# oxfordcontrol/COSMO.jl

Measured on AMD Instinct MI355X. Metric: ADMM iterations/sec (fp64) at fixed (n,m,nnz,cone), higher is better.
Workload: dtype f64

## Files before the change

cosmo.jl_amd/csrc/psd_polar.hip:

```cpp
#include "psd_internal.h"
#include <math.h>
#include <stdlib.h>
#include <string.h>
#include <algorithm>
#include <mutex>

#define PK 16
#ifndef POLAR_PREFETCH_DEPTH
#define POLAR_PREFETCH_DEPTH 2
#endif
#define PLD 80

struct PolarCone {
  int idx;
  int off, d, kind;
  int ts;
  int sk;
  int skg, skc;
  int ld;
  long long woff;
};

struct BatchCone { long long woff; int off, d, kind, ld, idx, ts; };

// ... 25 lines not shown
  real* W = nullptr;
  real* parts = nullptr;
  real* nrm = nullptr;
  int k_lift = REAL_IS_FLOAT ? 5 : 9;
  int max_rounds = 2;
  int rescale = 1;
  int batch_occ = 3;
  real tol_factor = 8.0;
  PolarDev* dev = nullptr;
  PolarDev seen;
  long long launches[4] = {0, 0, 0, 0};
  int streamk = 0;
  real* sk_scratch = nullptr;
  SkSync* sk_sync = nullptr;
  int sk_gmax = 0;
  unsigned sk_base = 0, sk_epoch = 0;
  int products_last_large = 0, products_last_batch = 0;
  std::vector<BatchCone> bcones;
  BatchCone* d_bcones = nullptr;
  int4* d_btiles = nullptr;
  int nbtiles = 0, nbtiles96 = 0;
  int speculate = 0;
  int* gate_host = nullptr;
  int batch_wave = 0;
  int batch_ragged = 1;
  void* d_rtiles = nullptr;
  int nrtiles = 0;
  int dataflow = 0;
  void* d_df_tiles = nullptr;
  int* d_df_cone_nt = nullptr;
  unsigned* d_df_sync = nullptr;
  int df_xoff[9] = {0, 0, 0, 0, 0, 0, 0, 0, 0};
  int df_grid = 0;
  long long df_launches = 0, df_timed = 0;
  int df_nprod = 0;
  double df_seconds = 0.0;
  hipEvent_t df_ev[2] = {nullptr, nullptr};
  int df_ev_pending = 0;
  void* h_rtiles = nullptr;
  void* rep_host = nullptr;
  void* d_rtiles_rep = nullptr;
  int nrep = 0;
  long long repair_launch_tiles = 0, repair_trains = 0;
  double batch_flops_performed = 0.0, batch_flops_useful = 0.0;
  int batch_ts96 = 0;
  real* BW = nullptr;
  real* bparts = nullptr;
  real* bnrm = nullptr;
  int* bgate = nullptr;
  int adapt = 0;
  int compact_repair = 1;
  std::vector<int> bk, bstreak, bm;
  int* d_lgate = nullptr;
  int* d_ubuf = nullptr;
  int* bgate_host = nullptr;
  int lgate_kmax = -1;
  long long depth_fail = 0, depth_down = 0, depth_proj = 0;
  int seen_proj_batch = 0;
  std::vector<int> lk, lstreak, lm;
  int seen_proj_large = 0;
  double wprod_last = 0.0;
};
#define POLAR_LIFT_CAP 18

extern "C" int32_t cosmo_hip_polar_schedule(int32_t k_lift, double* abc, int32_t* nsteps) {
  if (k_lift < 0 || k_lift > 64 || !nsteps) return COSMO_HIP_ERR_INVALID;
// ... 513 lines not shown
  t_first = RT_NOW();
#endif
  if (DEPTH == 1) {
    for (int kb = 0; kb + 1 < nk; kb += 2) {
      R_LOAD(r[0], kb + 1)
      R_COMPUTE(0)
      R_STORE(r[0], 1)
      __syncthreads();
      if (kb + 2 >= nk) break;
      R_LOAD(r[0], kb + 2)
      R_COMPUTE(1)
      R_STORE(r[0], 0)
      __syncthreads();
    }
  } else
  for (int kb = 0; kb + 1 < nk; kb += 2) {
    if (kb + 2 < nk) R_LOAD(r[0], kb + 2)
    R_COMPUTE(0)
    R_STORE(r[DEPTH - 1], 1)
    __syncthreads();
    if (kb + 2 >= nk) break;
    if (kb + 3 < nk) R_LOAD(r[DEPTH - 1], kb + 3)
    R_COMPUTE(1)
    R_STORE(r[0], 0)
    __syncthreads();
  }
  pre_last();
  if ((nk - 1) & 1) R_COMPUTE(1) else R_COMPUTE(0)
#undef R_LOAD
#undef R_STORE
#undef R_COMPUTE
}

template <int EPI, int OCC, bool SC1 = false, class Hook>
__device__ __forceinline__ void ragged_tile(const RTile& td, real* __restrict__ W, int ia, int ib, int icin, int ic, real alpha, real beta, real* smem, Hook pre_last) {
  const unsigned long long t_start = RT_NOW();
  unsigned long long t_first = t_start;
  (void)t_first;
#ifdef POLAR_LAB_TIMING
  const unsigned long long w_start = (threadIdx.x == 0) ? wall_clock64() : 0ull;
#endif
  const int ld = td.ld;
  const long long n2 = (long long)ld * ld;
  real* base = W + td.woff;
  const real* A = base + ia * n2;
  const real* B = base + ib * n2;
  const real* Cin = base + icin * n2;
  real* C = base + ic * n2;
  const int ei = td.ext & 255, ej = (td.ext >> 8) & 255, diag = (td.ext >> 16) & 1;
  const int nblk = diag ? ei * (ei + 1) / 2 : ei * ej;
  const int wv = __builtin_amdgcn_readfirstlane(threadIdx.x >> 6), lane = threadIdx.x & 63;
  int oa[4], ob[4];
  int nsl = 0;
#pragma unroll
  for (int sl = 0; sl < 4; ++sl) {
    const int q = wv + 4 * sl;
    int bi = 0, bj = 0;
    if (q < nblk) {
      nsl = sl + 1;
      if (diag) { bj = (q >= 6) ? 3 : (q >= 3) ? 2 : (q >= 1) ? 1 : 0; bi = q - bj * (bj + 1) / 2; }
      else { bj = q / ei; bi = q - bj * ei; }
    }
    oa[sl] = 16 * bi; ob[sl] = 16 * bj;
  }
  v4d acc[4];
#pragma unroll
// ... 3 lines not shown
  const int i0 = td.i0, j0 = td.j0;
  __amdgpu_buffer_rsrc_t rs = __builtin_amdgcn_make_buffer_rsrc((void*)base, 0, SC1 ? (int)(4 * n2 * (long long)sizeof(real)) : 0, 0x00020000);
  const int offA = (int)(ia * n2) + td.i0, offB = (int)(ib * n2) + td.j0;
#ifndef POLAR_LAB_NO_MAINLOOP
#define R_MAINLOOP(NSL_, SAME_) symm_mainloop_r<NSL_, (OCC >= 4 ? 1 : 2), SC1, SAME_>(A, B, ld, i0, j0, nk, smem, acc, oa, ob, pre_last, rs, offA, offB RT_ARG)
#ifndef POLAR_LAB_TWO_PANELS
  if (diag && offA == offB) {
    switch (nsl) {
      case 3: R_MAINLOOP(3, true); break;
      case 2: R_MAINLOOP(2, true); break;
      case 1: R_MAINLOOP(1, true); break;
      default: R_MAINLOOP(0, true); break;
    }
  } else
#endif
  switch (nsl) {
    case 4: R_MAINLOOP(4, false); break;
    case 3: R_MAINLOOP(3, false); break;
    case 2: R_MAINLOOP(2, false); break;
    case 1: R_MAINLOOP(1, false); break;
    default: R_MAINLOOP(0, false); break;
  }
#undef R_MAINLOOP
#else
  (void)A; (void)B; (void)nk; (void)pre_last;
#endif
#ifdef POLAR_LAB_NO_EPILOGUE
  if (lane == 0) C[(long long)j0 * ld + i0 + wv] = acc[0][0] + acc[1][0] + acc[2][0] + acc[3][0];
  return;
#endif
  const unsigned long long t_main = RT_NOW();
  (void)t_main; (void)t_start;
  (void)xi; (void)xj;
  {
    const int lj = lane & 15;
#pragma unroll
    for (int sl = 0; sl < 4; ++sl) {
      if (sl < nsl) {
        const int j = ob[sl] + lj;
        const bool dblk = diag && (oa[sl] == ob[sl]);
        real v[4];
        if (EPI == 1) {
          real c[4];
#pragma unroll
          for (int q = 0; q < 4; ++q) {
            const int i = oa[sl] + ACC_ROW(lane, q);
            const bool ok = !(dblk && i > j);
            const real* cp = Cin + (ok ? (long long)(i0 + i) * ld + j0 + j : 0);
            c[q] = SC1 ? __hip_atomic_load(cp, __ATOMIC_RELAXED, __HIP_MEMORY_SCOPE_AGENT) : *cp;
            if (!ok) c[q] = R(0.0);
          }
#pragma unroll
          for (int q = 0; q < 4; ++q) v[q] = alpha * acc[sl][q] + beta * c[q];
        } else {
#pragma unroll
          for (int q = 0; q < 4; ++q) v[q] = acc[sl][q];
        }
#pragma unroll
        for (int q = 0; q < 4; ++q) {
          const int i = oa[sl] + ACC_ROW(lane, q);
          if (!(dblk && i > j)) C[(long long)(j0 + j) * ld + i0 + i] = v[q];
        }
#pragma unroll
        for (int q = 0; q < 4; ++q) {
          const int i = oa[sl] + ACC_ROW(lane, q);
          if (!(dblk && i >= j)) C[(long long)(i0 + i) * ld + j0 + j] = v[q];
        }
      }
    }
  }
#ifdef POLAR_LAB_TIMING
  { const unsigned long long t_end = RT_NOW();
    RT_ADD(0, t_start); RT_ADD(1, t_first); RT_ADD(2, t_main); RT_ADD(3, t_end); RT_ADD(4, nk);
    if (threadIdx.x == 0 && blockIdx.x < RT_MAXT) g_rtw[blockIdx.x] = wall_clock64() - w_start; }
#endif
}

template <int EPI, int OCC>
__global__ __launch_bounds__(256) __attribute__((amdgpu_waves_per_eu(OCC, OCC))) void k_symm_gemm_batch_r(const Ctl* __restrict__ ctl, int guard, const int* __restrict__ gate,
                                                         const RTile* __restrict__ tiles, const BatchCone* __restrict__ cones, real* __restrict__ W,
                                                         int ia, int ib, int icin, int ic, real alpha, real beta) {
  extern __shared__ real smem[];
  const RTile td = tiles[blockIdx.x];
  const int halted = guard ? ctl->halt : 0;
  if (halted) return;
  if (td.cone < 0) return;
  if (gate && !gate[td.cone]) return;
  (void)cones;
  ragged_tile<EPI, OCC>(td, W, ia, ib, icin, ic, alpha, beta, smem, []() {});
}

struct DfProd { int ia, ib, icin, ic, epi, pad; real alpha, beta; };
#define DF_MAX_PROD 64
struct DfArgs { DfProd prod[DF_MAX_PROD]; int nprod; int xoff[9]; };
#define DF_SYNC_DONE 144
__device__ __forceinline__ unsigned df_xcc_id() { unsigned x; asm volatile("s_getreg_b32 %0, hwreg(HW_REG_XCC_ID)" : "=s"(x)); return x & 7u; }
__device__ __forceinline__ unsigned df_ld(const unsigned* p) { return __hip_atomic_load(p, __ATOMIC_RELAXED, __HIP_MEMORY_SCOPE_AGENT); }
#define DF_RMW(ptr) __hip_atomic_fetch_add((ptr), 1u, __ATOMIC_RELAXED, __HIP_MEMORY_SCOPE_AGENT)
template <int OCC>
__global__ __launch_bounds__(256) __attribute__((amdgpu_waves_per_eu(OCC, OCC))) void k_polar_dataflow(Ctl* __restrict__ ctl, int guard, const RTile* __restrict__ tiles,
                                                         const int* __restrict__ cone_nt, unsigned* __restrict__ sync, real* __restrict__ W, const DfArgs a) {
  extern __shared__ real smem[];
  __shared__ unsigned s_item;
  __shared__ int s_fail;
  if (guard && ctl->halt) return;
  const int x = (int)df_xcc_id();
  const int x0 = a.xoff[x];
  const unsigned n_x = (unsigned)(a.xoff[x + 1] - x0);
  const unsigned total = n_x * (unsigned)a.nprod;
  const bool wave0 = __builtin_amdgcn_readfirstlane(threadIdx.x >> 6) == 0;
  if (wave0) { if (threadIdx.x == 0) { s_fail = 0; s_item = (n_x > 0) ? DF_RMW(sync + 16 * x) : 0u; } }
  int prev_cone = -1;
  unsigned nxt = 0;
  bool first = true;
  for (;;) {
    if (wave0) {
      if (threadIdx.x == 0) {
        if (prev_cone >= 0) (void)DF_RMW(sync + DF_SYNC_DONE + prev_cone);
        if (!first) s_item = nxt;
      }
    }
    first = false;
    __syncthreads();
    const unsigned item = __builtin_amdgcn_readfirstlane(s_item);
    if (item >= total) break;
    const unsigned p = item / n_x, t = item - p * n_x;
    const RTile td = tiles[x0 + t];
    if (p > 0) {
      if (wave0) {
        if (threadIdx.x == 0) {
          const unsigned target = p * (unsigned)cone_nt[td.cone];
          const unsigned* cnt = sync + DF_SYNC_DONE + td.cone;
          long sp = 0;
          while (df_ld(cnt) < target) {
            __builtin_amdgcn_s_sleep(1);
            ++sp;
            if ((sp & 255) == 0 && df_ld(sync + 128)) { s_fail = 1; break; }
            if (sp > (1L << 20)) { s_fail = 1; __hip_atomic_store(sync + 128, 1u, __ATOMIC_RELAXED, __HIP_MEMORY_SCOPE_AGENT); ctl->error = COSMO_HIP_ERR_HIP; break; }
          }
        }
      }
      __syncthreads();
      if (__builtin_amdgcn_readfirstlane(s_fail)) break;
    }
    const DfProd pr = a.prod[p];
    auto hook = [&]() { if (wave0) { if (threadIdx.x == 0) nxt = DF_RMW(sync + 16 * x); } };
    if (pr.epi) ragged_tile<1, OCC, true>(td, W, pr.ia, pr.ib, pr.icin, pr.ic, pr.alpha, pr.beta, smem, hook);
    else ragged_tile<0, OCC, true>(td, W, pr.ia, pr.ib, pr.icin, pr.ic, pr.alpha, pr.beta, smem, hook);
    asm volatile("s_waitcnt vmcnt(0)" ::: "memory");
    __syncthreads();
    prev_cone = td.cone;
  }
}
#ifdef POLAR_LAB_TIMING
}
extern "C" void cosmo_dbg_ragged_timing(unsigned long long* out ) {
  (void)hipDeviceSynchronize();
  (void)hipMemcpyFromSymbol(out, HIP_SYMBOL(g_rt), sizeof(unsigned long long) * RT_MAXT * 5);
}
extern "C" void cosmo_dbg_ragged_wall(unsigned long long* out ) {
  (void)hipDeviceSynchronize();
  (void)hipMemcpyFromSymbol(out, HIP_SYMBOL(g_rtw), sizeof(unsigned long long) * RT_MAXT);
}
namespace {
#endif

#define WT_DEPTH 4
#define WT_SPITCH 66
template <int EPI>
__global__ __launch_bounds__(64) __attribute__((amdgpu_waves_per_eu(2, 2))) void k_symm_gemm_batch_w(const Ctl* __restrict__ ctl, int guard, const int* __restrict__ gate,
                                                         const int4* __restrict__ tiles, const BatchCone* __restrict__ cones, real* __restrict__ W,
                                                         int ia, int ib, int icin, int ic, real alpha, real beta) {
  if (guard && ctl->halt) return;
  const int4 td = tiles[blockIdx.x];
  if (td.x < 0) return;
  if (gate && !gate[td.x]) return;
  __shared__ real strip[16 * WT_SPITCH];
  const BatchCone bc = cones[td.x];
  const int ld = bc.ld;
  const long long n2 = (long long)ld * ld;
  real* base = W + bc.woff;
  const real* __restrict__ A = base + ia * n2;
  const real* __restrict__ B = base + ib * n2;
  const real* __restrict__ Cin = base + icin * n2;
  real* __restrict__ C = base + ic * n2;
// ... 423 lines not shown
      std::vector<int4> tl;
      if (getenv("COSMO_HIP_POLAR_BATCH_FLAT")) {
        for (int ci : order) {
          if (q->bcones[ci].ts != ts) continue;
          const int nt = q->bcones[ci].ld / ts;
          for (int tj = 0; tj < nt; ++tj) for (int ti = 0; ti <= tj; ++ti) tl.push_back(int4{ci, ti, tj, 0});
        }
      } else {
        std::vector<std::vector<int4>> xl(8);
        long long load[8] = {0, 0, 0, 0, 0, 0, 0, 0};
        for (int ci : order) {
          if (q->bcones[ci].ts != ts) continue;
          const int nt = q->bcones[ci].ld / ts;
          int x = 0;
          for (int t = 1; t < 8; ++t) if (load[t] < load[x]) x = t;
          for (int tj = 0; tj < nt; ++tj) for (int ti = 0; ti <= tj; ++ti) xl[x].push_back(int4{ci, ti, tj, 0});
          load[x] += (long long)nt * (nt + 1) / 2 * q->bcones[ci].ld;
        }
        size_t maxlen = 0;
        for (int x = 0; x < 8; ++x) maxlen = std::max(maxlen, xl[x].size());
        tl.assign(8 * maxlen, int4{-1, 0, 0, 0});
        for (int x = 0; x < 8; ++x) for (size_t sl = 0; sl < xl[x].size(); ++sl) tl[8 * sl + x] = xl[x][sl];
      }
      count[cls] = (int)tl.size();
      tiles.insert(tiles.end(), tl.begin(), tl.end());
    }
    q->nbtiles = count[0]; q->nbtiles96 = count[1];
    if (const char* e = getenv("COSMO_HIP_POLAR_BATCH_RAGGED")) q->batch_ragged = atoi(e) ? 1 : 0;
    if (q->batch_ts96 || q->batch_wave) q->batch_ragged = 0;
    q->batch_flops_performed = q->batch_flops_useful = 0.0;
    for (const BatchCone& bc : q->bcones) q->batch_flops_useful += (double)bc.d * bc.d * (bc.d + 1.0);
    if (q->batch_ragged) {
      std::vector<std::vector<RTile>> xl(8);
      long long load[8] = {0, 0, 0, 0, 0, 0, 0, 0};
      for (int ci : order) {
        const BatchCone& bc = q->bcones[ci];
        const int nb16 = (bc.d + 15) / 16, nt = (nb16 + 3) / 4;
        std::vector<int> start(nt + 1, 0);
        for (int t = 0; t < nt; ++t) start[t + 1] = start[t] + nb16 / nt + (t < nb16 % nt ? 1 : 0);
        int x = 0;
        for (int t = 1; t < 8; ++t) if (load[t] < load[x]) x = t;
        for (int tj = 0; tj < nt; ++tj)
          for (int ti = 0; ti <= tj; ++ti) {
            const int ei = start[ti + 1] - start[ti], ej = start[tj + 1] - start[tj], dg = (ti == tj) ? 1 : 0;
            RTile rt; rt.cone = ci; rt.i0 = 16 * start[ti]; rt.j0 = 16 * start[tj]; rt.ext = ei | (ej << 8) | (dg << 16);
            rt.ld = bc.ld; rt.d = bc.d; rt.woff = bc.woff;
            if (rt.i0 + 64 > bc.ld || rt.j0 + 64 > bc.ld) return cosmo_fail(h, COSMO_HIP_ERR_INVALID, "ragged tile exceeds the leading dimension");
            xl[x].push_back(rt);
            const int nblk = dg ? ei * (ei + 1) / 2 : ei * ej, slots = (nblk + 3) / 4;
            load[x] += (long long)slots * nb16;
            q->batch_flops_performed += 2.0 * 256.0 * nblk * 16.0 * nb16;
          }
      }
      int sort_tiles = 1;
      if (const char* e = getenv("COSMO_HIP_POLAR_BATCH_SORT")) sort_tiles = atoi(e) ? 1 : 0;
      if (sort_tiles) {
        auto cost = [](const RTile& t) {
          const int ei = t.ext & 255, ej = (t.ext >> 8) & 255, dg = (t.ext >> 16) & 1;
          const int nblk = dg ? ei * (ei + 1) / 2 : ei * ej, slots = (nblk + 3) / 4;
          return (long long)((t.d + 15) / 16) * (10 * slots + 2) + 125;
        };
        for (int x = 0; x < 8; ++x) std::stable_sort(xl[x].begin(), xl[x].end(), [&](const RTile& a, const RTile& b) { return cost(a) > cost(b); });
      }
      size_t maxlen = 0;
      for (int x = 0; x < 8; ++x) maxlen = std::max(maxlen, xl[x].size());
      std::vector<RTile> rl(8 * std::max<size_t>(maxlen, 1), RTile{-1, 0, 0, 0, 0, 0, 0});
      for (int x = 0; x < 8; ++x) for (size_t sl = 0; sl < xl[x].size(); ++sl) rl[8 * sl + x] = xl[x][sl];
      q->nrtiles = (int)rl.size();
      {
        std::vector<RTile> dl;
        std::vector<int> cnt(q->bcones.size(), 0);
        for (int x = 0; x < 8; ++x) { q->df_xoff[x] = (int)dl.size(); for (const RTile& t : xl[x]) { dl.push_back(t); cnt[(size_t)t.cone] += 1; } }
        q->df_xoff[8] = (int)dl.size();
        if (dl.empty()) dl.push_back(RTile{-1, 0, 0, 0, 0, 0, 0});
        HIPCHK(h, hipMalloc((void**)&q->d_df_tiles, sizeof(RTile) * dl.size()));
        HIPCHK(h, hipMemcpy(q->d_df_tiles, dl.data(), sizeof(RTile) * dl.size(), hipMemcpyHostToDevice));
        HIPCHK(h, hipMalloc((void**)&q->d_df_cone_nt, sizeof(int) * std::max<size_t>(cnt.size(), 1)));
        HIPCHK(h, hipMemcpy(q->d_df_cone_nt, cnt.data(), sizeof(int) * cnt.size(), hipMemcpyHostToDevice));
        HIPCHK(h, hipMalloc((void**)&q->d_df_sync, sizeof(unsigned) * (DF_SYNC_DONE + cnt.size())));
        hipDeviceProp_t prop;
        HIPCHK(h, hipGetDeviceProperties(&prop, h->device));
        q->df_grid = std::max(1, prop.multiProcessorCount) * 4;
        { int nmin = INT32_MAX; for (int x = 0; x < 8; ++x) nmin = std::min(nmin, q->df_xoff[x + 1] - q->df_xoff[x]); q->dataflow = (nmin >= q->df_grid / 8) ? 1 : 0; }
        if (const char* e = getenv("COSMO_HIP_POLAR_DATAFLOW")) q->dataflow = atoi(e) ? 1 : 0;
        if (const char* e = getenv("COSMO_HIP_POLAR_DATAFLOW_GRID")) { const int v = atoi(e); if (v >= 8 && v <= 8192) q->df_grid = v; }
        (void)hipFuncSetAttribute((const void*)k_polar_dataflow<4>, hipFuncAttributeMaxDynamicSharedMemorySize, GemmCfg<64>::SMEM); }
      HIPCHK(h, hipMalloc((void**)&q->d_rtiles, sizeof(RTile) * rl.size()));
      HIPCHK(h, hipMemcpy(q->d_rtiles, rl.data(), sizeof(RTile) * rl.size(), hipMemcpyHostToDevice));
      q->h_rtiles = malloc(sizeof(RTile) * rl.size());
      if (!q->h_rtiles) return cosmo_fail(h, COSMO_HIP_ERR_HIP, "out of host memory");
      memcpy(q->h_rtiles, rl.data(), sizeof(RTile) * rl.size());
      HIPCHK(h, hipMalloc((void**)&q->d_rtiles_rep, sizeof(RTile) * rl.size()));
      HIPCHK(h, hipHostMalloc((void**)&q->rep_host, sizeof(RTile) * rl.size()));
      (void)hipFuncSetAttribute((const void*)k_symm_gemm_batch_r<0, 3>, hipFuncAttributeMaxDynamicSharedMemorySize, GemmCfg<64>::SMEM);
      (void)hipFuncSetAttribute((const void*)k_symm_gemm_batch_r<1, 3>, hipFuncAttributeMaxDynamicSharedMemorySize, GemmCfg<64>::SMEM);
      (void)hipFuncSetAttribute((const void*)k_symm_gemm_batch_r<0, 4>, hipFuncAttributeMaxDynamicSharedMemorySize, GemmCfg<64>::SMEM);
      (void)hipFuncSetAttribute((const void*)k_symm_gemm_batch_r<1, 4>, hipFuncAttributeMaxDynamicSharedMemorySize, GemmCfg<64>::SMEM);
    } else {
      for (const BatchCone& bc : q->bcones) { const long long nt = bc.ld / bc.ts; q->batch_flops_performed += 2.0 * (double)(nt * (nt + 1) / 2) * bc.ts * bc.ts * (((bc.d + 31) / 32) * 32); }
    }
    if (tiles.empty()) tiles.push_back(int4{-1, 0, 0, 0});
    HIPCHK(h, hipMalloc((void**)&q->BW, sizeof(real) * (size_t)woff));
    HIPCHK(h, hipMemset(q->BW, 0, sizeof(real) * (size_t)woff));
    HIPCHK(h, hipMalloc((void**)&q->d_bcones, sizeof(BatchCone) * q->bcones.size()));
    HIPCHK(h, hipMalloc((void**)&q->d_btiles, sizeof(int4) * tiles.size()));
    HIPCHK(h, hipMalloc((void**)&q->bparts, sizeof(real) * 3 * BPX * q->bcones.size()));
    HIPCHK(h, hipMalloc((void**)&q->bnrm, sizeof(real) * q->bcones.size()));
    HIPCHK(h, hipMalloc((void**)&q->bgate, sizeof(int) * q->bcones.size()));
    HIPCHK(h, hipMemset(q->bgate, 0, sizeof(int) * q->bcones.size()));
    { const size_t nb = q->bcones.size();
      { int pat = 3; if (const char* e = getenv("COSMO_HIP_POLAR_PATIENCE")) pat = std::max(1, atoi(e));
        q->bk.assign(nb, q->k_lift); q->bstreak.assign(nb, 0); q->bm.assign(nb, pat); }
      HIPCHK(h, hipMalloc((void**)&q->d_lgate, sizeof(int) * nb * POLAR_LIFT_CAP));
      HIPCHK(h, hipMalloc((void**)&q->d_ubuf, sizeof(int) * nb));
      HIPCHK(h, hipHostMalloc((void**)&q->bgate_host, sizeof(int) * nb, hipHostMallocDefault));
      q->lgate_kmax = -1; }
    HIPCHK(h, hipMemcpy(q->d_bcones, q->bcones.data(), sizeof(BatchCone) * q->bcones.size(), hipMemcpyHostToDevice));
    HIPCHK(h, hipMemcpy(q->d_btiles, tiles.data(), sizeof(int4) * tiles.size(), hipMemcpyHostToDevice));
    (void)hipFuncSetAttribute((const void*)k_symm_gemm_batch<0, 3, 64>, hipFuncAttributeMaxDynamicSharedMemorySize, GemmCfg<64>::SMEM);
// ... 65 lines not shown
        for (int t = t0; t < kmax; ++t) lg[(size_t)t * n + c] = 1;
        ub[(size_t)c] = (t0 & 1) ? 2 : 1;
      }
      HIPCHK(h, hipMemcpyAsync(q->d_lgate, lg.data(), sizeof(int) * lg.size(), hipMemcpyHostToDevice, st));
      HIPCHK(h, hipMemcpyAsync(q->d_ubuf, ub.data(), sizeof(int) * ub.size(), hipMemcpyHostToDevice, st));
      HIPCHK(h, hipStreamSynchronize(st));
      q->lgate_kmax = kmax;
    }
  }
  hipLaunchKernelGGL(k_bpolar_populate, dim3(BPX, n), dim3(COSMO_BS), 0, st, h->ctl, guard, q->d_bcones, s, q->BW, q->bparts);
  hipLaunchKernelGGL(k_bpolar_scale, dim3(BPX, n), dim3(COSMO_BS), 0, st, h->ctl, guard, q->d_bcones, q->bparts, q->BW, q->bnrm, adapt ? (const int*)q->d_ubuf : (const int*)nullptr);
  int iu = 1, iy = 2, products = 0;
  DfArgs dfa;
  bool df = q->dataflow && q->batch_ragged && q->nrtiles > 0 && !adapt && !h->profiling && 3 * (kmax + POLAR_NFIN) + 2 <= DF_MAX_PROD;
  dfa.nprod = 0;
  auto product = [&](int epi, const int* gate, int ia, int ib, int icin, int ic, real alpha, real beta) {
    if (df) { DfProd& pr = dfa.prod[dfa.nprod++]; pr.ia = ia; pr.ib = ib; pr.icin = icin; pr.ic = ic; pr.epi = epi; pr.pad = 0; pr.alpha = alpha; pr.beta = beta; return; }
    if (epi) launch_bgemm<1>(q, st, h->ctl, guard, gate, ia, ib, icin, ic, alpha, beta);
    else launch_bgemm<0>(q, st, h->ctl, guard, gate, ia, ib, icin, ic, alpha, beta);
  };
  auto flush_dataflow = [&]() -> int32_t {
    if (!df) return COSMO_HIP_OK;
    for (int x = 0; x < 9; ++x) dfa.xoff[x] = q->df_xoff[x];
    HIPCHK(h, hipMemsetAsync(q->d_df_sync, 0, sizeof(unsigned) * (DF_SYNC_DONE + q->bcones.size()), st));
    if (!q->df_ev[0]) { HIPCHK(h, hipEventCreate(&q->df_ev[0])); HIPCHK(h, hipEventCreate(&q->df_ev[1])); }
    if (q->df_ev_pending && hipEventQuery(q->df_ev[1]) == hipSuccess) {
      float ms = 0.f;
      if (hipEventElapsedTime(&ms, q->df_ev[0], q->df_ev[1]) == hipSuccess) { q->df_seconds += 1e-3 * (double)ms; q->df_timed += 1; }
      q->df_ev_pending = 0;
    }
    (void)hipGetLastError();
    const bool timed = !q->df_ev_pending;
    if (timed) HIPCHK(h, hipEventRecord(q->df_ev[0], st));
    hipLaunchKernelGGL((k_polar_dataflow<4>), dim3(q->df_grid), dim3(256), GemmCfg<64>::SMEM, st, h->ctl, guard, (const RTile*)q->d_df_tiles, (const int*)q->d_df_cone_nt,
                       q->d_df_sync, q->BW, dfa);
    if (timed) { HIPCHK(h, hipEventRecord(q->df_ev[1], st)); q->df_ev_pending = 1; }
    q->df_launches += 1; q->df_nprod = dfa.nprod;
    df = false;
    return COSMO_HIP_OK;
  };
  auto step = [&](const real* co, const int* gate) {
    product(0, gate, iu, iu, iu, iy, 1.0, 0.0);
    product(1, gate, iy, iy, iy, 3, co[2], co[1]);
    product(1, gate, iu, 3, iu, iy, 1.0, co[0]);
    std::swap(iu, iy);
    products += 3; q->launches[3] += 3;
  };
  auto verify = [&](int round, const int* gate) -> int32_t {
    product(0, gate, iu, 0, 0, 3, 1.0, 0.0);
    product(1, gate, iu, 3, 0, iy, 1.0, -1.0);
    CHK(flush_dataflow());
    hipLaunchKernelGGL(k_bpolar_sumsq, dim3(BPX, n), dim3(COSMO_BS), 0, st, h->ctl, guard, gate, q->d_bcones, q->BW, iy, vparts);
    hipLaunchKernelGGL(k_bpolar_decide, dim3(1), dim3(COSMO_BS), 0, st, h->ctl, guard, q->dev, q->bgate, round, round == q->max_rounds ? 1 : 0, n, q->d_bcones,
                       vparts, q->bnrm, q->tol_factor);
    products += 2; q->launches[3] += 2;
    return COSMO_HIP_OK;
  };
  for (int t = 0; t < kmax; ++t) step(kPolarLift, adapt ? (const int*)(q->d_lgate + (size_t)t * n) : (const int*)nullptr);
  for (int t = 0; t < POLAR_NFIN; ++t) step(kPolarFinish[t], nullptr);
  CHK(verify(0, nullptr));
  q->products_last_batch = products;
  { double wsum = 0.0, w3 = 0.0;
    for (int c = 0; c < n; ++c) { const double d3 = (double)q->bcones[c].d * q->bcones[c].d * q->bcones[c].d; w3 += d3; wsum += d3 * (3.0 * ((adapt ? q->bk[c] : kmax) + POLAR_NFIN) + 2.0); }
    q->wprod_last = w3 > 0.0 ? wsum / w3 : 0.0; }
  for (int r = 1; r <= q->max_rounds; ++r) {
    if (!q->speculate) {
      HIPCHK(h, hipMemcpyAsync(q->gate_host, &q->dev->gate, (adapt && r == 1 ? 5 : 1) * sizeof(int), hipMemcpyDeviceToHost, st));
      if (r == 1 && q->bgate_host) HIPCHK(h, hipMemcpyAsync(q->bgate_host, q->bgate, sizeof(int) * (size_t)n, hipMemcpyDeviceToHost, st));
// ... 129 lines not shown

extern "C" int32_t cosmo_hip_polar_stats(cosmo_hip_handle* h, int64_t out[16]) {
  if (!h || !out) return COSMO_HIP_ERR_INVALID;
  for (int i = 0; i < 16; ++i) out[i] = 0;
  PolarPlan* q = static_cast<PolarPlan*>(h->psd_polar);
  if (!q) return COSMO_HIP_OK;
  if (hipSetDevice(h->device) != hipSuccess) return cosmo_fail(h, COSMO_HIP_ERR_HIP, "hipSetDevice failed");
  PolarDev now;
  HIPCHK(h, hipMemcpyAsync(&now, q->dev, sizeof now, hipMemcpyDeviceToHost, h->stream));
  HIPCHK(h, hipStreamSynchronize(h->stream));
  out[0] = (int64_t)q->cones.size(); out[1] = (int64_t)q->bcones.size();
  if (!q->cones.empty()) { out[2] = q->cones[0].ts; out[3] = q->cones[0].sk; }
  out[4] = q->launches[0]; out[5] = q->launches[1]; out[6] = q->launches[2]; out[7] = q->launches[3];
  out[8] = q->products_last_large; out[9] = now.rounds; out[10] = now.verified; out[11] = q->products_last_batch;
  out[12] = q->k_lift + POLAR_NFIN; out[13] = now.unverified; out[14] = now.projections;
  out[15] = (int64_t)llround((double)now.err_max * 1e18);
  return COSMO_HIP_OK;
}

extern "C" int32_t cosmo_hip_polar_dataflow_stats(cosmo_hip_handle* h, double out[8]) {
  if (!h || !out) return COSMO_HIP_ERR_INVALID;
  for (int i = 0; i < 8; ++i) out[i] = 0.0;
  PolarPlan* q = static_cast<PolarPlan*>(h->psd_polar);
  if (!q) return COSMO_HIP_OK;
  if (hipSetDevice(h->device) != hipSuccess) return cosmo_fail(h, COSMO_HIP_ERR_HIP, "hipSetDevice failed");
  if (q->df_ev_pending) {
    HIPCHK(h, hipEventSynchronize(q->df_ev[1]));
    float ms = 0.f;
    if (hipEventElapsedTime(&ms, q->df_ev[0], q->df_ev[1]) == hipSuccess) { q->df_seconds += 1e-3 * (double)ms; q->df_timed += 1; }
    q->df_ev_pending = 0;
  }
  out[0] = q->dataflow; out[1] = (double)q->df_launches; out[2] = q->df_nprod; out[3] = (double)q->df_timed;
  out[4] = q->df_timed ? q->df_seconds / (double)q->df_timed : 0.0;
  out[5] = q->batch_flops_performed * q->df_nprod; out[6] = q->df_grid; out[7] = q->df_xoff[8];
  return COSMO_HIP_OK;
}
extern "C" int32_t cosmo_hip_polar_dataflow_reset_timing(cosmo_hip_handle* h) {
  if (!h) return COSMO_HIP_ERR_INVALID;
  PolarPlan* q = static_cast<PolarPlan*>(h->psd_polar);
  if (q) { q->df_seconds = 0.0; q->df_timed = 0; }
  return COSMO_HIP_OK;
}

extern "C" int32_t cosmo_hip_polar_depth_stats(cosmo_hip_handle* h, int64_t out[8]) {
  if (!h || !out) return COSMO_HIP_ERR_INVALID;
  for (int i = 0; i < 8; ++i) out[i] = 0;
  PolarPlan* q = static_cast<PolarPlan*>(h->psd_polar);
  if (!q) return COSMO_HIP_OK;
  const bool adapt = q->adapt && !q->speculate && !getenv("COSMO_HIP_POLAR_KLIFT") && q->k_lift <= POLAR_LIFT_CAP;
  out[0] = adapt ? 1 : 0;
  const std::vector<int>& ks = !q->bk.empty() ? q->bk : q->lk;
  if (adapt && !ks.empty()) {
    long long sum = 0; int mn = ks[0], mx = ks[0];
    for (int v : ks) { sum += v; mn = std::min(mn, v); mx = std::max(mx, v); }
    out[1] = mn; out[2] = mx; out[3] = (1000 * sum) / (long long)ks.size();
  } else { out[1] = out[2] = q->k_lift; out[3] = 1000LL * q->k_lift; }
  out[4] = (int64_t)llround(1000.0 * q->wprod_last);
  out[5] = q->depth_fail; out[6] = q->depth_down; out[7] = q->depth_proj;
  return COSMO_HIP_OK;
}

extern "C" int32_t cosmo_hip_polar_streamk_stats(cosmo_hip_handle* h, int64_t out[4]) {
  if (!h || !out) return COSMO_HIP_ERR_INVALID;
  for (int i = 0; i < 4; ++i) out[i] = 0;
  PolarPlan* q = static_cast<PolarPlan*>(h->psd_polar);
  if (!q || q->cones.empty() || !q->sk_sync) return COSMO_HIP_OK;
  if (hipSetDevice(h->device) != hipSuccess) return cosmo_fail(h, COSMO_HIP_ERR_HIP, "hipSetDevice failed");
// ... 107 lines not shown
```

Baseline: 365.2.

## Pair adjacent symmetric tiles into 512-thread dataflow blocks sharing A panels

Adds a paired dataflow kernel in which each 512-thread block computes two output tiles of the same cone, normally tiles in one row with adjacent columns. Both tiles share the same A panel, so it is loaded into LDS once and only the distinct panels (at most three) are staged. The goal is to cut global loads and per-item scheduling overhead in the polar-iteration products. The new path is on by default (df_pair=3), and odd leftover tiles are paired across rows. In exchange the block uses more LDS and twice the threads, which may lower occupancy, and the rule that enables dataflow mode changes.

```diff
diff --git a/cosmo.jl_amd/csrc/psd_polar.hip b/cosmo.jl_amd/csrc/psd_polar.hip
--- a/cosmo.jl_amd/csrc/psd_polar.hip
+++ b/cosmo.jl_amd/csrc/psd_polar.hip
@@ -81,6 +81,8 @@
   unsigned* d_df_sync = nullptr;
   int df_xoff[9] = {0, 0, 0, 0, 0, 0, 0, 0, 0};
   int df_grid = 0;
+  int df_pair = 3;
+  int df_ntiles = 0;
   long long df_launches = 0, df_timed = 0;
   int df_nprod = 0;
   double df_seconds = 0.0;
@@ -660,6 +662,46 @@
 #undef R_COMPUTE
 }
 
+template <int EPI, bool SC1>
+__device__ __forceinline__ void ragged_store(const v4d (&acc)[4], const int (&oa)[4], const int (&ob)[4], int nsl, int diag, int i0, int j0, int ld,
+                                             const real* __restrict__ Cin, real* __restrict__ C, real alpha, real beta, int lane) {
+  const int lj = lane & 15;
+#pragma unroll
+  for (int sl = 0; sl < 4; ++sl) {
+    if (sl < nsl) {
+      const int j = ob[sl] + lj;
+      const bool dblk = diag && (oa[sl] == ob[sl]);
+      real v[4];
+      if (EPI == 1) {
+        real c[4];
+#pragma unroll
+        for (int q = 0; q < 4; ++q) {
+          const int i = oa[sl] + ACC_ROW(lane, q);
+          const bool ok = !(dblk && i > j);
+          const real* cp = Cin + (ok ? (long long)(i0 + i) * ld + j0 + j : 0);
+          c[q] = SC1 ? __hip_atomic_load(cp, __ATOMIC_RELAXED, __HIP_MEMORY_SCOPE_AGENT) : *cp;
+          if (!ok) c[q] = R(0.0);
+        }
+#pragma unroll
+        for (int q = 0; q < 4; ++q) v[q] = alpha * acc[sl][q] + beta * c[q];
+      } else {
+#pragma unroll
+        for (int q = 0; q < 4; ++q) v[q] = acc[sl][q];
+      }
+#pragma unroll
+      for (int q = 0; q < 4; ++q) {
+        const int i = oa[sl] + ACC_ROW(lane, q);
+        if (!(dblk && i > j)) C[(long long)(j0 + j) * ld + i0 + i] = v[q];
+      }
+#pragma unroll
+      for (int q = 0; q < 4; ++q) {
+        const int i = oa[sl] + ACC_ROW(lane, q);
+        if (!(dblk && i >= j)) C[(long long)(i0 + i) * ld + j0 + j] = v[q];
+      }
+    }
+  }
+}
+
 template <int EPI, int OCC, bool SC1 = false, class Hook>
 __device__ __forceinline__ void ragged_tile(const RTile& td, real* __restrict__ W, int ia, int ib, int icin, int ic, real alpha, real beta, real* smem, Hook pre_last) {
   const unsigned long long t_start = RT_NOW();
@@ -729,43 +771,7 @@
   const unsigned long long t_main = RT_NOW();
   (void)t_main; (void)t_start;
   (void)xi; (void)xj;
-  {
-    const int lj = lane & 15;
-#pragma unroll
-    for (int sl = 0; sl < 4; ++sl) {
-      if (sl < nsl) {
-        const int j = ob[sl] + lj;
-        const bool dblk = diag && (oa[sl] == ob[sl]);
-        real v[4];
-        if (EPI == 1) {
-          real c[4];
-#pragma unroll
-          for (int q = 0; q < 4; ++q) {
-            const int i = oa[sl] + ACC_ROW(lane, q);
-            const bool ok = !(dblk && i > j);
-            const real* cp = Cin + (ok ? (long long)(i0 + i) * ld + j0 + j : 0);
-            c[q] = SC1 ? __hip_atomic_load(cp, __ATOMIC_RELAXED, __HIP_MEMORY_SCOPE_AGENT) : *cp;
-            if (!ok) c[q] = R(0.0);
-          }
-#pragma unroll
-          for (int q = 0; q < 4; ++q) v[q] = alpha * acc[sl][q] + beta * c[q];
-        } else {
-#pragma unroll
-          for (int q = 0; q < 4; ++q) v[q] = acc[sl][q];
-        }
-#pragma unroll
-        for (int q = 0; q < 4; ++q) {
-          const int i = oa[sl] + ACC_ROW(lane, q);
-          if (!(dblk && i > j)) C[(long long)(j0 + j) * ld + i0 + i] = v[q];
-        }
-#pragma unroll
-        for (int q = 0; q < 4; ++q) {
-          const int i = oa[sl] + ACC_ROW(lane, q);
-          if (!(dblk && i >= j)) C[(long long)(i0 + i) * ld + j0 + j] = v[q];
-        }
-      }
-    }
-  }
+  ragged_store<EPI, SC1>(acc, oa, ob, nsl, diag, i0, j0, ld, Cin, C, alpha, beta, lane);
 #ifdef POLAR_LAB_TIMING
   { const unsigned long long t_end = RT_NOW();
     RT_ADD(0, t_start); RT_ADD(1, t_first); RT_ADD(2, t_main); RT_ADD(3, t_end); RT_ADD(4, nk);
@@ -794,12 +800,134 @@
 __device__ __forceinline__ unsigned df_xcc_id() { unsigned x; asm volatile("s_getreg_b32 %0, hwreg(HW_REG_XCC_ID)" : "=s"(x)); return x & 7u; }
 __device__ __forceinline__ unsigned df_ld(const unsigned* p) { return __hip_atomic_load(p, __ATOMIC_RELAXED, __HIP_MEMORY_SCOPE_AGENT); }
 #define DF_RMW(ptr) __hip_atomic_fetch_add((ptr), 1u, __ATOMIC_RELAXED, __HIP_MEMORY_SCOPE_AGENT)
-template <int OCC>
-__global__ __launch_bounds__(256) __attribute__((amdgpu_waves_per_eu(OCC, OCC))) void k_polar_dataflow(Ctl* __restrict__ ctl, int guard, const RTile* __restrict__ tiles,
-                                                         const int* __restrict__ cone_nt, unsigned* __restrict__ sync, real* __restrict__ W, const DfArgs a) {
-  extern __shared__ real smem[];
-  __shared__ unsigned s_item;
-  __shared__ int s_fail;
+
+struct alignas(16) RPair { int cone; int i0, j0, i1, j1; int ext0, ext1; int ld, d; int pad; long long woff; };
+
+template <int NSL, class PreLast>
+__device__ __forceinline__ void pair_mainloop(int ld, int nk, real* smem, v4d (&acc)[4], const int (&oa)[4], const int (&ob)[4], const real* aimg, const real* bimg,
+                                              PreLast pre_last, __amdgpu_buffer_rsrc_t rs, int off0, int off1, int off2, bool ld1, bool ld2) {
+  using Cfg = GemmCfg<64>;
+  constexpr int PITCH = Cfg::PITCH, PANEL = Cfg::PANEL;
+  real* P0s = smem;
+  real* P1s = P0s + 2 * PANEL;
+  real* P2s = P0s + 4 * PANEL;
+  int tid = (int)threadIdx.x;
+  asm volatile("" : "+v"(tid));
+  const int lane = tid & 63;
+  const int pstep = PK * ld;
+  const int goff = (tid / 32) * ld + 2 * (tid % 32), soff = (tid / 32) * PITCH + 2 * (tid % 32);
+  real2 r[3] = {make_real2(R(0.0), R(0.0)), make_real2(R(0.0), R(0.0)), make_real2(R(0.0), R(0.0))};
+#define P_LOAD(KB)                                                                                        \
+  {                                                                                                       \
+    const int o_ = (KB) * pstep + goff;                                                                   \
+    r[0] = polar_ld_pair_sc1(rs, (off0 + o_) * (int)sizeof(real));                                        \
+    if (ld1) r[1] = polar_ld_pair_sc1(rs, (off1 + o_) * (int)sizeof(real));                              \
+    if (ld2) r[2] = polar_ld_pair_sc1(rs, (off2 + o_) * (int)sizeof(real));                              \
+  }
+#define P_STORE(BUF)                                                                                      \
+  {                                                                                                       \
+    real* pa_ = P0s + (BUF) * PANEL + soff;                                                                \
+    pa_[0] = r[0].x; pa_[1] = r[0].y;                                                                     \
+    if (ld1) { real* pb_ = P1s + (BUF) * PANEL + soff; pb_[0] = r[1].x; pb_[1] = r[1].y; }                \
+    if (ld2) { real* pb_ = P2s + (BUF) * PANEL + soff; pb_[0] = r[2].x; pb_[1] = r[2].y; }                \
+  }
+  const int fl = lane & 15, fk = lane >> 4;
+  const real* apb[4]; const real* bpb[4];
+#pragma unroll
+  for (int sl = 0; sl < 4; ++sl) { apb[sl] = aimg + fk * PITCH + fl + oa[sl]; bpb[sl] = bimg + fk * PITCH + fl + ob[sl]; }
+#define P_COMPUTE(BUF)                                                                                   \
+  {                                                                                                       \
+    _Pragma("unroll") for (int ks = 0; ks < PK / 4; ++ks) {                                               \
+      real av[NSL > 0 ? NSL : 1], bv[NSL > 0 ? NSL : 1];                                                  \
+      _Pragma("unroll") for (int sl = 0; sl < NSL; ++sl) {                                                \
+        av[sl] = FRAG_RD(apb[sl] + (BUF) * PANEL + ks * 4 * PITCH);                                       \
+        bv[sl] = FRAG_RD(bpb[sl] + (BUF) * PANEL + ks * 4 * PITCH);                                       \
+      }                                                                                                   \
+      _Pragma("unroll") for (int sl = 0; sl < NSL; ++sl) acc[sl] = MFMA_REAL(av[sl], bv[sl], acc[sl]);    \
+    }                                                                                                     \
+  }
+  P_LOAD(0)
+  P_STORE(0)
+  __syncthreads();
+  for (int kb = 0; kb + 1 < nk; kb += 2) {
+    P_LOAD(kb + 1)
+    P_COMPUTE(0)
+    P_STORE(1)
+    __syncthreads();
+    if (kb + 2 >= nk) break;
+    P_LOAD(kb + 2)
+    P_COMPUTE(1)
+    P_STORE(0)
+    __syncthreads();
+  }
+  pre_last();
+  if ((nk - 1) & 1) P_COMPUTE(1) else P_COMPUTE(0)
+#undef P_LOAD
+#undef P_STORE
+#undef P_COMPUTE
+}
+
+template <int EPI, class Hook>
+__device__ __forceinline__ void paired_item(const RPair& td, real* __restrict__ W, int ia, int ib, int icin, int ic, real alpha, real beta, real* smem, Hook pre_last) {
+  constexpr int PANEL = GemmCfg<64>::PANEL;
+  const int ld = td.ld;
+  const long long n2 = (long long)ld * ld;
+  real* base = W + td.woff;
+  const real* Cin = base + icin * n2;
+  real* C = base + ic * n2;
+  const int wv8 = __builtin_amdgcn_readfirstlane(threadIdx.x >> 6), lane = threadIdx.x & 63;
+  const int half = wv8 >> 2, wv = wv8 & 3;
+  const int ext = half ? td.ext1 : td.ext0, j0 = half ? td.j1 : td.j0, i0 = half ? td.i1 : td.i0;
+  const int ei = ext & 255, ej = (ext >> 8) & 255, diag = (ext >> 16) & 1;
+  const int nblk = diag ? ei * (ei + 1) / 2 : ei * ej;
+  int oa[4], ob[4];
+  int nsl = 0;
+#pragma unroll
+  for (int sl = 0; sl < 4; ++sl) {
+    const int q = wv + 4 * sl;
+    int bi = 0, bj = 0;
+    if (q < nblk) {
+      nsl = sl + 1;
+      if (diag) { bj = (q >= 6) ? 3 : (q >= 3) ? 2 : (q >= 1) ? 1 : 0; bi = q - bj * (bj + 1) / 2; }
+      else { bj = q / ei; bi = q - bj * ei; }
+    }
+    oa[sl] = 16 * bi; ob[sl] = 16 * bj;
+  }
+  v4d acc[4];
+#pragma unroll
+  for (int sl = 0; sl < 4; ++sl) acc[sl] = v4d{0.0, 0.0, 0.0, 0.0};
+  const int nk = ((td.d + 15) / 16);
+  __amdgpu_buffer_rsrc_t rs = __builtin_amdgcn_make_buffer_rsrc((void*)base, 0, (int)(4 * n2 * (long long)sizeof(real)), 0x00020000);
+  int off[3] = {(int)(ia * n2) + td.i0, 0, 0};
+  int np = 1;
+  auto slot = [&](int o) {
+    if (o == off[0]) return 0;
+    if (np > 1 && o == off[1]) return 1;
+    if (np > 2 && o == off[2]) return 2;
+    if (np < 3) { off[np] = o; return np++; }
+    return 2;
+  };
+  const int sb0 = slot((int)(ib * n2) + td.j0);
+  int sa1 = 0, sb1 = 0;
+  if (td.ext1) { sa1 = slot((int)(ia * n2) + td.i1); sb1 = slot((int)(ib * n2) + td.j1); }
+  const bool ld1 = np > 1, ld2 = np > 2;
+  const real* aimg = smem + 2 * PANEL * (half ? sa1 : 0);
+  const real* bimg = smem + 2 * PANEL * (half ? sb1 : sb0);
+#define P_MAINLOOP(NSL_) pair_mainloop<NSL_>(ld, nk, smem, acc, oa, ob, aimg, bimg, pre_last, rs, off[0], off[1], off[2], ld1, ld2)
+  switch (nsl) {
+    case 4: P_MAINLOOP(4); break;
+    case 3: P_MAINLOOP(3); break;
+    case 2: P_MAINLOOP(2); break;
+    case 1: P_MAINLOOP(1); break;
+    default: P_MAINLOOP(0); break;
+  }
+#undef P_MAINLOOP
+  ragged_store<EPI, true>(acc, oa, ob, nsl, diag, i0, j0, ld, Cin, C, alpha, beta, lane);
+}
+
+template <int OCC, bool PAIR, class Item>
+__device__ __forceinline__ void polar_dataflow_loop(Ctl* __restrict__ ctl, int guard, const Item* __restrict__ tiles, const int* __restrict__ cone_nt,
+                                                    unsigned* __restrict__ sync, real* __restrict__ W, const DfArgs& a, real* smem, unsigned& s_item, int& s_fail) {
   if (guard && ctl->halt) return;
   const int x = (int)df_xcc_id();
   const int x0 = a.xoff[x];
@@ -822,7 +950,7 @@
     const unsigned item = __builtin_amdgcn_readfirstlane(s_item);
     if (item >= total) break;
     const unsigned p = item / n_x, t = item - p * n_x;
-    const RTile td = tiles[x0 + t];
+    const Item td = tiles[x0 + t];
     if (p > 0) {
       if (wave0) {
         if (threadIdx.x == 0) {
@@ -842,12 +970,34 @@
     }
     const DfProd pr = a.prod[p];
     auto hook = [&]() { if (wave0) { if (threadIdx.x == 0) nxt = DF_RMW(sync + 16 * x); } };
-    if (pr.epi) ragged_tile<1, OCC, true>(td, W, pr.ia, pr.ib, pr.icin, pr.ic, pr.alpha, pr.beta, smem, hook);
-    else ragged_tile<0, OCC, true>(td, W, pr.ia, pr.ib, pr.icin, pr.ic, pr.alpha, pr.beta, smem, hook);
+    if constexpr (PAIR) {
+      if (pr.epi) paired_item<1>(td, W, pr.ia, pr.ib, pr.icin, pr.ic, pr.alpha, pr.beta, smem, hook);
+      else paired_item<0>(td, W, pr.ia, pr.ib, pr.icin, pr.ic, pr.alpha, pr.beta, smem, hook);
+    } else {
+      if (pr.epi) ragged_tile<1, OCC, true>(td, W, pr.ia, pr.ib, pr.icin, pr.ic, pr.alpha, pr.beta, smem, hook);
+      else ragged_tile<0, OCC, true>(td, W, pr.ia, pr.ib, pr.icin, pr.ic, pr.alpha, pr.beta, smem, hook);
+    }
     asm volatile("s_waitcnt vmcnt(0)" ::: "memory");
     __syncthreads();
     prev_cone = td.cone;
   }
+}
+template <int OCC>
+__global__ __launch_bounds__(256) __attribute__((amdgpu_waves_per_eu(OCC, OCC))) void k_polar_dataflow(Ctl* __restrict__ ctl, int guard, const RTile* __restrict__ tiles,
+                                                         const int* __restrict__ cone_nt, unsigned* __restrict__ sync, real* __restrict__ W, const DfArgs a) {
+  extern __shared__ real smem[];
+  __shared__ unsigned s_item;
+  __shared__ int s_fail;
+  polar_dataflow_loop<OCC, false>(ctl, guard, tiles, cone_nt, sync, W, a, smem, s_item, s_fail);
+}
+#define DF_PAIR_SMEM (6 * GemmCfg<64>::PANEL * (int)sizeof(real))
+template <int OCC>
+__global__ __launch_bounds__(512) __attribute__((amdgpu_waves_per_eu(OCC, OCC))) void k_polar_dataflow_pair(Ctl* __restrict__ ctl, int guard, const RPair* __restrict__ tiles,
+                                                         const int* __restrict__ cone_nt, unsigned* __restrict__ sync, real* __restrict__ W, const DfArgs a) {
+  extern __shared__ real smem[];
+  __shared__ unsigned s_item;
+  __shared__ int s_fail;
+  polar_dataflow_loop<OCC, true>(ctl, guard, tiles, cone_nt, sync, W, a, smem, s_item, s_fail);
 }
 #ifdef POLAR_LAB_TIMING
 }
@@ -1337,6 +1487,8 @@
     for (const BatchCone& bc : q->bcones) q->batch_flops_useful += (double)bc.d * bc.d * (bc.d + 1.0);
     if (q->batch_ragged) {
       std::vector<std::vector<RTile>> xl(8);
+      std::vector<std::vector<RPair>> xp(8);
+      if (const char* e = getenv("COSMO_HIP_POLAR_PAIRED")) { const int v = atoi(e); if (v >= 0 && v <= 3) q->df_pair = v; }
       long long load[8] = {0, 0, 0, 0, 0, 0, 0, 0};
       for (int ci : order) {
         const BatchCone& bc = q->bcones[ci];
@@ -1356,6 +1508,26 @@
             load[x] += (long long)slots * nb16;
             q->batch_flops_performed += 2.0 * 256.0 * nblk * 16.0 * nb16;
           }
+        auto item = [&](int ti, int tj, int ti1, int tj1) {
+          auto ext = [&](int a, int b) { return (start[a + 1] - start[a]) | ((start[b + 1] - start[b]) << 8) | ((a == b ? 1 : 0) << 16); };
+          RPair it; it.cone = ci; it.i0 = 16 * start[ti]; it.j0 = 16 * start[tj]; it.ld = bc.ld; it.d = bc.d; it.woff = bc.woff; it.pad = 0;
+          it.ext0 = ext(ti, tj);
+          it.i1 = ti1 >= 0 ? 16 * start[ti1] : it.i0; it.j1 = ti1 >= 0 ? 16 * start[tj1] : it.j0;
+          it.ext1 = ti1 >= 0 ? ext(ti1, tj1) : 0;
+          xp[x].push_back(it);
+        };
+        if (q->df_pair == 2) { for (int tj = 0; tj < nt; ++tj) for (int ti = 0; ti <= tj; ++ti) item(ti, tj, -1, -1); }
+        else {
+          int left = -1;
+          for (int ti = 0; ti < nt; ++ti)
+            for (int tj = ti; tj < nt; tj += 2) {
+              if (tj + 1 < nt) item(ti, tj, ti, tj + 1);
+              else if (q->df_pair != 3) item(ti, tj, -1, -1);
+              else if (left < 0) left = ti;
+              else { item(left, tj, ti, tj); left = -1; }
+            }
+          if (left >= 0) item(left, nt - 1, -1, -1);
+        }
       }
       int sort_tiles = 1;
       if (const char* e = getenv("COSMO_HIP_POLAR_BATCH_SORT")) sort_tiles = atoi(e) ? 1 : 0;
@@ -1366,6 +1538,14 @@
           return (long long)((t.d + 15) / 16) * (10 * slots + 2) + 125;
         };
         for (int x = 0; x < 8; ++x) std::stable_sort(xl[x].begin(), xl[x].end(), [&](const RTile& a, const RTile& b) { return cost(a) > cost(b); });
+        auto pcost = [&](const RPair& it) {
+          RTile t; t.d = it.d; t.ext = it.ext0;
+          const long long c0 = cost(t);
+          if (!it.ext1) return c0;
+          t.ext = it.ext1;
+          return std::max(c0, cost(t));
+        };
+        for (int x = 0; x < 8; ++x) std::stable_sort(xp[x].begin(), xp[x].end(), [&](const RPair& a, const RPair& b) { return pcost(a) > pcost(b); });
       }
       size_t maxlen = 0;
       for (int x = 0; x < 8; ++x) maxlen = std::max(maxlen, xl[x].size());
@@ -1373,23 +1553,36 @@
       for (int x = 0; x < 8; ++x) for (size_t sl = 0; sl < xl[x].size(); ++sl) rl[8 * sl + x] = xl[x][sl];
       q->nrtiles = (int)rl.size();
       {
-        std::vector<RTile> dl;
         std::vector<int> cnt(q->bcones.size(), 0);
-        for (int x = 0; x < 8; ++x) { q->df_xoff[x] = (int)dl.size(); for (const RTile& t : xl[x]) { dl.push_back(t); cnt[(size_t)t.cone] += 1; } }
-        q->df_xoff[8] = (int)dl.size();
-        if (dl.empty()) dl.push_back(RTile{-1, 0, 0, 0, 0, 0, 0});
-        HIPCHK(h, hipMalloc((void**)&q->d_df_tiles, sizeof(RTile) * dl.size()));
-        HIPCHK(h, hipMemcpy(q->d_df_tiles, dl.data(), sizeof(RTile) * dl.size(), hipMemcpyHostToDevice));
+        q->df_ntiles = 0;
+        for (int x = 0; x < 8; ++x) q->df_ntiles += (int)xl[x].size();
+        if (q->df_pair) {
+          std::vector<RPair> dl;
+          for (int x = 0; x < 8; ++x) { q->df_xoff[x] = (int)dl.size(); for (const RPair& t : xp[x]) { dl.push_back(t); cnt[(size_t)t.cone] += 1; } }
+          q->df_xoff[8] = (int)dl.size();
+          if (dl.empty()) dl.push_back(RPair{-1, 0, 0, 0, 0, 0, 0, 0, 0, 0, 0});
+          HIPCHK(h, hipMalloc((void**)&q->d_df_tiles, sizeof(RPair) * dl.size()));
+          HIPCHK(h, hipMemcpy(q->d_df_tiles, dl.data(), sizeof(RPair) * dl.size(), hipMemcpyHostToDevice));
+        } else {
+          std::vector<RTile> dl;
+          for (int x = 0; x < 8; ++x) { q->df_xoff[x] = (int)dl.size(); for (const RTile& t : xl[x]) { dl.push_back(t); cnt[(size_t)t.cone] += 1; } }
+          q->df_xoff[8] = (int)dl.size();
+          if (dl.empty()) dl.push_back(RTile{-1, 0, 0, 0, 0, 0, 0});
+          HIPCHK(h, hipMalloc((void**)&q->d_df_tiles, sizeof(RTile) * dl.size()));
+          HIPCHK(h, hipMemcpy(q->d_df_tiles, dl.data(), sizeof(RTile) * dl.size(), hipMemcpyHostToDevice));
+        }
         HIPCHK(h, hipMalloc((void**)&q->d_df_cone_nt, sizeof(int) * std::max<size_t>(cnt.size(), 1)));
         HIPCHK(h, hipMemcpy(q->d_df_cone_nt, cnt.data(), sizeof(int) * cnt.size(), hipMemcpyHostToDevice));
         HIPCHK(h, hipMalloc((void**)&q->d_df_sync, sizeof(unsigned) * (DF_SYNC_DONE + cnt.size())));
         hipDeviceProp_t prop;
         HIPCHK(h, hipGetDeviceProperties(&prop, h->device));
+        const int slots = std::max(1, prop.multiProcessorCount) * (q->df_pair ? 2 : 4);
         q->df_grid = std::max(1, prop.multiProcessorCount) * 4;
-        { int nmin = INT32_MAX; for (int x = 0; x < 8; ++x) nmin = std::min(nmin, q->df_xoff[x + 1] - q->df_xoff[x]); q->dataflow = (nmin >= q->df_grid / 8) ? 1 : 0; }
+        { int nmin = INT32_MAX; for (int x = 0; x < 8; ++x) nmin = std::min(nmin, q->df_xoff[x + 1] - q->df_xoff[x]); q->dataflow = (nmin >= slots / 8) ? 1 : 0; }
         if (const char* e = getenv("COSMO_HIP_POLAR_DATAFLOW")) q->dataflow = atoi(e) ? 1 : 0;
         if (const char* e = getenv("COSMO_HIP_POLAR_DATAFLOW_GRID")) { const int v = atoi(e); if (v >= 8 && v <= 8192) q->df_grid = v; }
-        (void)hipFuncSetAttribute((const void*)k_polar_dataflow<4>, hipFuncAttributeMaxDynamicSharedMemorySize, GemmCfg<64>::SMEM); }
+        (void)hipFuncSetAttribute((const void*)k_polar_dataflow<4>, hipFuncAttributeMaxDynamicSharedMemorySize, GemmCfg<64>::SMEM);
+        (void)hipFuncSetAttribute((const void*)k_polar_dataflow_pair<4>, hipFuncAttributeMaxDynamicSharedMemorySize, DF_PAIR_SMEM); }
       HIPCHK(h, hipMalloc((void**)&q->d_rtiles, sizeof(RTile) * rl.size()));
       HIPCHK(h, hipMemcpy(q->d_rtiles, rl.data(), sizeof(RTile) * rl.size(), hipMemcpyHostToDevice));
       q->h_rtiles = malloc(sizeof(RTile) * rl.size());
@@ -1521,8 +1714,12 @@
     (void)hipGetLastError();
     const bool timed = !q->df_ev_pending;
     if (timed) HIPCHK(h, hipEventRecord(q->df_ev[0], st));
-    hipLaunchKernelGGL((k_polar_dataflow<4>), dim3(q->df_grid), dim3(256), GemmCfg<64>::SMEM, st, h->ctl, guard, (const RTile*)q->d_df_tiles, (const int*)q->d_df_cone_nt,
-                       q->d_df_sync, q->BW, dfa);
+    if (q->df_pair)
+      hipLaunchKernelGGL((k_polar_dataflow_pair<4>), dim3(q->df_grid), dim3(512), DF_PAIR_SMEM, st, h->ctl, guard, (const RPair*)q->d_df_tiles, (const int*)q->d_df_cone_nt,
+                         q->d_df_sync, q->BW, dfa);
+    else
+      hipLaunchKernelGGL((k_polar_dataflow<4>), dim3(q->df_grid), dim3(256), GemmCfg<64>::SMEM, st, h->ctl, guard, (const RTile*)q->d_df_tiles, (const int*)q->d_df_cone_nt,
+                         q->d_df_sync, q->BW, dfa);
     if (timed) { HIPCHK(h, hipEventRecord(q->df_ev[1], st)); q->df_ev_pending = 1; }
     q->df_launches += 1; q->df_nprod = dfa.nprod;
     df = false;
@@ -1718,7 +1915,7 @@
   }
   out[0] = q->dataflow; out[1] = (double)q->df_launches; out[2] = q->df_nprod; out[3] = (double)q->df_timed;
   out[4] = q->df_timed ? q->df_seconds / (double)q->df_timed : 0.0;
-  out[5] = q->batch_flops_performed * q->df_nprod; out[6] = q->df_grid; out[7] = q->df_xoff[8];
+  out[5] = q->batch_flops_performed * q->df_nprod; out[6] = q->df_grid; out[7] = q->df_ntiles;
   return COSMO_HIP_OK;
 }
 extern "C" int32_t cosmo_hip_polar_dataflow_reset_timing(cosmo_hip_handle* h) {
```

Result: faster. 373.0, median of 6 (+2.1%).
